# svohr/mixemt

Hardware: AMD Instinct MI355X
Metric: read x hap cells/sec through the EM iteration (EM iters/sec reported beside it as em_iters_per_s), 1000000 reads x 5408 haps in total, whole job (higher is better)
Workload: dtype f64

## Files before the change

### include/mixemt_hip_tuning.h

```cpp
#ifndef MIXEMT_HIP_TUNING_H
#define MIXEMT_HIP_TUNING_H

#include <stddef.h>
#include <stdint.h>

#ifdef __cplusplus
extern "C" {
#endif

struct mxm_em_state;

int mxm_reset_tuning(void);

int mxm_set_timing_events(void *ev_start, void *ev_stop);

int mxm_describe_stream_kernel(int32_t H, int32_t nb, char *buf, size_t len);

int mxm_diag_stream_read(const void *src, size_t bytes, int32_t wg_per_cu, int32_t blocked,
                         void *sink, void *stream);

struct mxm_coded;
int mxm_diag_stream_coded(const struct mxm_coded *c, int32_t H, int32_t wg_per_cu, void *sink, void *stream);

int mxm_diag_stream_quads(const struct mxm_coded *c, int32_t H, int32_t wg_per_cu, void *sink, void *stream);

int mxm_set_progress_callback(void (*fn)(const struct mxm_em_state *state_host, int32_t B, void *user),
                              void *user, int32_t every);

int mxm_set_loop_graph(int32_t mode);

int mxm_set_loop_fused(int32_t mode, int32_t chunk);

int mxm_set_fused_coded_grid(int32_t nwg);

int mxm_set_quad_left_grid(int32_t nwg);

int mxm_set_sparse_long_rows(int32_t on);
int mxm_set_sparse_long_entries(int32_t n);

int mxm_set_quad_encoder(int32_t kind);

int mxm_set_coded_batch_tile(int32_t bt);

int mxm_diag_fused_force_abort(int32_t on);

int mxm_diag_fused_stamps(const void *ws, unsigned long long *out_host);

int mxm_set_batch_tile(int32_t bt);

int mxm_set_compact_restarts(int32_t mode);

#define MXM_SAMPLES_TILE_ROWS 32
int mxm_samples_tile_rows(void);

int mxm_set_min_rows_per_wg(int32_t n);

int mxm_set_sparse_max_distinct(int32_t n);

#ifdef __cplusplus
}
#endif
#endif
```

### mixemt_amd/_lib.py

```python

import ctypes
import os

_PKG = os.path.dirname(os.path.abspath(__file__))
LIB_PATH = os.environ.get("MXM_LIB") or os.path.join(_PKG, "lib", "libmixemt_hip.so")

c_i32, c_i64, c_f64 = ctypes.c_int32, ctypes.c_int64, ctypes.c_double
c_ptr, c_size = ctypes.c_void_p, ctypes.c_size_t


class EmState(ctypes.Structure):
    _fields_ = [("done", c_i32), ("iters", c_i32), ("l1", c_f64), ("ticket", ctypes.c_uint32), ("error", ctypes.c_uint32)]


class Coded(ctypes.Structure):
    _fields_ = [("rec", c_ptr), ("rec_off", c_ptr), ("ndist", c_ptr), ("R", c_i64),
                ("P_rest", c_ptr), ("ldp_rest", c_i64), ("w_rest", c_ptr), ("R_rest", c_i64),
                ("wide_rows", c_ptr), ("n_wide", c_i64),
                ("qrec", c_ptr), ("qoff", c_ptr), ("nquad", c_ptr), ("quad_rows", c_ptr), ("n_quad_rows", c_i64),
                ("byte_rows", c_ptr), ("n_byte_rows", c_i64)]


class SampleTile(ctypes.Structure):
    _fields_ = [("sample", c_i32), ("count", c_i32), ("first", c_i64)]
# ... 80 lines not shown
                                         ctypes.POINTER(EmState)]),
    "mxm_samples_tile_rows": (ctypes.c_int, []),
    "mxm_samples_plan": (c_i64, [c_ptr, c_i32, c_ptr, c_i64, c_ptr]),
    "mxm_samples_workspace_bytes": (c_size, [c_i64, c_i32, c_i32]),
    "mxm_em_iter_samples": (ctypes.c_int, [ctypes.POINTER(Coded), c_ptr, c_i32, c_ptr, c_ptr, c_i32, c_ptr, c_ptr, c_ptr,
                                           c_size, c_ptr]),
    "mxm_em_loop_samples": (ctypes.c_int, [ctypes.POINTER(Coded), c_ptr, c_i32, c_ptr, c_i32, c_ptr, c_ptr, c_ptr, c_ptr,
                                           c_ptr, c_f64, c_i32, c_i32, c_ptr, c_size, c_ptr, ctypes.POINTER(EmState)]),
    "mxm_em_step": (ctypes.c_int, [c_ptr, c_i64, c_ptr, c_ptr, c_i64, c_i32, c_ptr, c_i64, c_i32,
                                   c_ptr, c_ptr, c_size, c_ptr]),
    "mxm_log_normalize": (ctypes.c_int, [c_ptr, c_i32, c_ptr, c_ptr]),
    "mxm_l1_exp_diff": (ctypes.c_int, [c_ptr, c_ptr, c_i32, c_ptr, c_ptr]),
    "mxm_add_scalar": (ctypes.c_int, [c_ptr, c_i64, c_i64, c_i32, c_f64, c_ptr]),
    "mxm_assign_reads": (ctypes.c_int, [c_ptr, c_i64, c_ptr, c_ptr, c_i32, c_i64, c_i32, c_f64, c_ptr, c_ptr]),
    "mxm_diag_stream_read": (ctypes.c_int, [c_ptr, c_size, c_i32, c_i32, c_ptr, c_ptr]),
    "mxm_diag_stream_coded": (ctypes.c_int, [ctypes.POINTER(Coded), c_i32, c_i32, c_ptr, c_ptr]),
    "mxm_diag_stream_quads": (ctypes.c_int, [ctypes.POINTER(Coded), c_i32, c_i32, c_ptr, c_ptr]),
    "mxm_diag_fused_force_abort": (ctypes.c_int, [c_i32]),
    "mxm_set_fused_coded_grid": (ctypes.c_int, [c_i32]),
    "mxm_set_quad_left_grid": (ctypes.c_int, [c_i32]),
    "mxm_set_coded_batch_tile": (ctypes.c_int, [c_i32]),
    "mxm_set_sparse_long_rows": (ctypes.c_int, [c_i32]),
    "mxm_set_quad_encoder": (ctypes.c_int, [c_i32]),
    "mxm_set_sparse_long_entries": (ctypes.c_int, [c_i32]),
    "mxm_diag_fused_stamps": (ctypes.c_int, [c_ptr, ctypes.POINTER(ctypes.c_ulonglong)]),
    "mxm_set_timing_events": (ctypes.c_int, [c_ptr, c_ptr]),
    "mxm_set_batch_tile": (ctypes.c_int, [c_i32]),
    "mxm_encode_signatures": (ctypes.c_int64, [ctypes.c_char_p, c_ptr, c_i64, c_ptr, c_i64, c_ptr, c_ptr, c_ptr,
                                               c_i64]),
    "mxm_aln_encode": (ctypes.c_int, [ctypes.POINTER(AlnColumns), c_ptr, c_i64, c_ptr, c_i32, c_i32, c_i32, c_i32,
                                      ctypes.POINTER(c_ptr)]),
    "mxm_aln_sizes_of": (ctypes.c_int, [c_ptr, ctypes.POINTER(AlnSizes)]),
    "mxm_aln_fetch": (ctypes.c_int, [c_ptr, c_ptr, c_ptr, c_ptr, c_ptr, c_ptr, c_ptr, c_ptr, c_ptr, c_ptr]),
    "mxm_aln_fetch_fragments": (ctypes.c_int, [c_ptr, c_ptr, c_ptr, c_ptr, c_ptr]),
    "mxm_aln_free": (None, [c_ptr]),
    "mxm_bam_read": (ctypes.c_int, [ctypes.c_char_p, c_i32, ctypes.POINTER(c_ptr)]),
    "mxm_bam_sizes_of": (ctypes.c_int, [c_ptr, ctypes.POINTER(BamSizes)]),
    "mxm_bam_columns": (ctypes.c_int, [c_ptr, ctypes.POINTER(AlnColumns)]),
    "mxm_bam_fetch_names": (ctypes.c_int, [c_ptr, c_ptr, c_ptr, c_ptr, c_ptr]),
    "mxm_bam_free": (None, [c_ptr]),
    "mxm_observe_bases": (ctypes.c_int, [ctypes.POINTER(AlnColumns), c_ptr, c_i32, c_i32, c_i64, c_ptr, c_ptr]),
    "mxm_observe_bases_labelled": (ctypes.c_int, [ctypes.POINTER(AlnColumns), c_ptr, c_ptr, c_i32, c_i32, c_i32, c_i64,
                                                  c_ptr, c_ptr]),
    "mxm_consensus": (ctypes.c_int, [c_ptr, c_i32, c_i64, c_i64, c_i64, c_i32, c_ptr, c_ptr, c_ptr, c_ptr]),
    "mxm_new_variants": (ctypes.c_int, [c_ptr, c_i64, c_i32, ctypes.POINTER(c_i32), c_i32, c_i64, c_ptr, c_ptr, c_ptr]),
    "mxm_first_observed": (ctypes.c_int, [ctypes.POINTER(AlnColumns), c_ptr, c_ptr, c_i32, c_i32, c_i32, c_i64, c_ptr,
                                          c_ptr, c_ptr]),
    "mxm_extend_assign": (ctypes.c_int, [ctypes.POINTER(AlnColumns), c_ptr, c_ptr, c_i32, c_i32, ctypes.POINTER(c_i32),
                                         c_i32, c_i32, c_i32, c_i32, c_ptr, c_i64, c_ptr, c_ptr, c_ptr, c_ptr]),
    "mxm_set_compact_restarts": (ctypes.c_int, [c_i32]),
    "mxm_set_loop_graph": (ctypes.c_int, [c_i32]),
    "mxm_set_loop_fused": (ctypes.c_int, [c_i32, c_i32]),
    "mxm_set_progress_callback": (ctypes.c_int, [c_ptr, c_ptr, c_i32]),
    "mxm_set_min_rows_per_wg": (ctypes.c_int, [c_i32]),
    "mxm_reset_tuning": (ctypes.c_int, []),
    "mxm_describe_stream_kernel": (ctypes.c_int, [c_i32, c_i32, ctypes.c_char_p, c_size]),
    "mxm_set_sparse_max_distinct": (ctypes.c_int, [c_i32]),
    "mxm_row_argmax_votes": (ctypes.c_int, [c_ptr, c_i64, c_ptr, c_i64, c_i32, c_ptr, c_ptr,
                                            c_ptr, c_size, c_ptr]),
    "mxm_first_seen": (ctypes.c_int, [c_ptr, c_i64, c_i32, c_ptr, c_ptr]),
    "mxm_gather_columns": (ctypes.c_int, [c_ptr, c_i64, c_i64, c_i32, c_ptr, c_i32, c_ptr, c_i64, c_ptr]),
    "mxm_fold_logaddexp": (ctypes.c_int, [c_ptr, c_i64, ctypes.POINTER(c_ptr), ctypes.POINTER(c_i64), c_i32,
                                          c_i64, c_i32, c_f64, c_ptr]),
}

FINISH_SIGNATURES = {
    "mxm_samples_finish_workspace_bytes": (c_size, [c_i64, c_i32, c_i32]),
    "mxm_votes_samples": (ctypes.c_int, [ctypes.POINTER(Coded), c_ptr, c_i32, c_i32, c_ptr, c_ptr, c_ptr, c_ptr, c_ptr, c_ptr,
                                         c_ptr, c_ptr, c_ptr, c_ptr, c_ptr, c_size, c_ptr]),
    "mxm_gather_columns_samples": (ctypes.c_int, [ctypes.POINTER(Coded), c_ptr, c_i32, c_i32, c_ptr, c_ptr, c_i32, c_ptr,
                                                  c_ptr, c_size, c_ptr]),
    "mxm_em_loop_samples_narrow": (ctypes.c_int, [ctypes.POINTER(Coded), c_ptr, c_i32, c_i32, c_ptr, c_i32, c_ptr, c_ptr,
                                                  c_ptr, c_ptr, c_ptr, c_ptr, c_f64, c_i32, c_i32, c_ptr, c_ptr, c_size,
                                                  c_ptr, ctypes.POINTER(EmState)]),
    "mxm_assign_reads_samples": (ctypes.c_int, [ctypes.POINTER(Coded), c_ptr, c_i32, c_i32, c_ptr, c_i32, c_ptr, c_ptr,
                                                c_ptr, c_ptr, c_ptr, c_ptr, c_f64, c_ptr, c_ptr, c_ptr, c_size, c_ptr]),
}

VARCHECK_SIGNATURES = {
    "mxm_check_variants_samples": (ctypes.c_int, [c_ptr, c_i32, c_i64, c_ptr, c_ptr, c_i32, c_ptr, c_ptr, c_i32, c_i64, c_ptr,
                                                  c_ptr, c_i32, c_f64, c_f64, c_f64, c_i32, c_i32, c_ptr, c_ptr, c_ptr, c_ptr]),
}

ABI_VERSION = 603

PROGRESS_FN = ctypes.CFUNCTYPE(None, ctypes.POINTER(EmState), c_i32, c_ptr)

_lib = None


class MixemtHipError(RuntimeError):
    pass


def load():
    global _lib
    if _lib is not None:
        return _lib
    if not os.path.exists(LIB_PATH):
        raise MixemtHipError(
            "libmixemt_hip.so is not built (%s); run `python -m mixemt_amd.build` -- "
            "there is no CPU fallback for the EM hot path" % LIB_PATH)
    from . import _dev
    lib = ctypes.CDLL(LIB_PATH)
    try:
        lib.mxm_version.restype = ctypes.c_int
        lib.mxm_version.argtypes = []
        have = lib.mxm_version()
    except AttributeError:
        have = None
    if have != ABI_VERSION:
        raise MixemtHipError("%s reports ABI version %s, this binding was written for %d: rebuild with "
                             "`python -m mixemt_amd.build --force`" % (LIB_PATH, have, ABI_VERSION))
    for name, (restype, argtypes) in (list(SIGNATURES.items()) + list(FINISH_SIGNATURES.items())
                                      + list(VARCHECK_SIGNATURES.items())):
        try:
            fn = getattr(lib, name)
        except AttributeError:
            raise MixemtHipError("%s has ABI version %d but lacks %s: rebuild with "
                                 "`python -m mixemt_amd.build --force`" % (LIB_PATH, have, name))
        fn.restype = restype
        fn.argtypes = argtypes
    _lib = lib
    try:
        if _dev.torch is not None and _dev.torch.cuda.is_available():
            lib.mxm_preload()
    except Exception:
        pass
    return lib


def check(rc, what):
    if rc != 0:
        msg = load().mxm_last_error().decode("utf-8", "replace")
        raise ValueError("%s failed (%d): %s" % (what, rc, msg))
```

### mixemt_amd/build.py

```python

import hashlib
import os
import shutil
import subprocess
import sys

_PKG = os.path.dirname(os.path.abspath(__file__))
_ROOT = os.path.dirname(_PKG)
SRC = os.path.join(_PKG, "csrc", "mixemt_hip.hip")
HDRS = [os.path.join(_ROOT, "include", name) for name in ("mixemt_hip.h", "mixemt_hip_tuning.h", "mixemt_hip_samples_finish.h",
                                                           "mixemt_hip_var_check.h")]
LIB_DIR = os.path.join(_PKG, "lib")
LIB = os.path.join(LIB_DIR, "libmixemt_hip.so")
ARCH = "gfx950"


def _hipcc():
    for cand in (os.environ.get("HIPCC"), shutil.which("hipcc"), "/opt/rocm/bin/hipcc"):
        if cand and os.path.exists(cand):
            return cand
    raise RuntimeError("hipcc not found (set HIPCC or add /opt/rocm/bin to PATH)")


def _sources():
    csrc = os.path.dirname(SRC)
    return sorted(os.path.join(csrc, f) for f in os.listdir(csrc) if f.endswith((".hip", ".hpp"))) + HDRS


def _digest(flags):
    h = hashlib.sha256()
    for path in _sources():
        with open(path, "rb") as fin:
            h.update(fin.read())
    h.update(" ".join(flags).encode())
    return h.hexdigest()


def build(force=False, defines=(), verbose=False, out=None):
    global LIB
    if out is not None:
        LIB = os.path.abspath(out)
    flags = ["--offload-arch=%s" % ARCH, "-O3", "-std=c++17", "-shared", "-fPIC", "-Werror=format",
             "-I" + os.path.join(_ROOT, "include"), "-I" + os.path.dirname(SRC)]
    flags += ["-D%s" % d for d in defines]
    stamp = LIB + ".stamp"
    want = _digest(flags)
    if not force and os.path.exists(LIB) and os.path.exists(stamp):
        with open(stamp) as fin:
            if fin.read().strip() == want:
                return LIB
    os.makedirs(os.path.dirname(LIB), exist_ok=True)
    cmd = [_hipcc()] + flags + [SRC, "-o", LIB, "-lz"]
    if verbose:
        sys.stderr.write(" ".join(cmd) + "\n")
    proc = subprocess.run(cmd, stdout=subprocess.PIPE, stderr=subprocess.STDOUT, text=True)
    if proc.returncode != 0:
        raise RuntimeError("hipcc failed:\n" + proc.stdout)
    with open(stamp, "w") as fout:
        fout.write(want + "\n")
    return LIB


if __name__ == "__main__":
    defs = []
    argv = sys.argv[1:]
    i = 0
    while i < len(argv):
        if argv[i] == "-D":
            defs.append(argv[i + 1])
            i += 2
        elif argv[i].startswith("-D"):
            defs.append(argv[i][2:])
            i += 1
        else:
            i += 1
    out_path = argv[argv.index("--out") + 1] if "--out" in argv else None
    print(build(force="--force" in argv, defines=defs, verbose=True, out=out_path))
```

### mixemt_amd/csrc/mixemt_hip.hip

```cpp
#include <hip/hip_runtime.h>
#include <stdint.h>
#include <stdio.h>
#include <stdlib.h>
#include <string.h>
#include <math.h>
#include <algorithm>
#include <atomic>
#include <mutex>
#include <type_traits>
#include <utility>
#include <vector>

#include "mixemt_hip.h"
#include "mixemt_hip_tuning.h"

#include "common.hpp"
#include "aln_encode.hpp"
#include "bam_reader.hpp"
#include "coded_kernels.hpp"
#include "quad_kernels.hpp"
#include "quad_batched_kernels.hpp"
#include "build_kernels.hpp"
#include "build_lut_kernels.hpp"
#include "build_sparse_kernels.hpp"
#include "em_kernels.hpp"
#include "estep_kernels.hpp"
#include "aux_kernels.hpp"
#include "records_kernels.hpp"
#include "fused_kernels.hpp"
#include "fused_cols_kernels.hpp"
#include "fused_coded_kernels.hpp"
#include "fused_narrow_kernels.hpp"
#include "samples_kernels.hpp"
#include "samples_finish_kernels.hpp"
#include "exchange.hpp"
#include "aln_walk.hpp"
#include "observe_kernels.hpp"
#include "var_check_kernels.hpp"
#include "assemble_kernels.hpp"


struct mxm_em_state;
typedef void (*mxm_progress_fn)(const mxm_em_state *state_host, int32_t B, void *user);
struct mxm_tuning {
    int sparse_maxd = -1;
    int min_rows_per_wg = 8;
    int compact_restarts = 2;
    int max_bt = 4;
    int loop_graph = -1;
    int loop_fused = -1;
    int fused_chunk = 0;
    int fused_cols = 1;
    int fused_coded_wg = 0;
    int quad_left_wg = 0;
    int sparse_long_entries = 5120;
    int quad_encoder = 1;
    int sparse_long = 1;
    int coded_bt = 3;
    int fused_force_abort = 0;
    double fused_cells = 1.0e8;
    hipEvent_t ev_start = nullptr, ev_stop = nullptr;
    mxm_progress_fn progress = nullptr;
    void *progress_user = nullptr;
    int progress_every = 10;
};
static std::mutex g_tune_mu;
static mxm_tuning g_tune;
static thread_local mxm_tuning T;
#define MXM_ENTER() do { std::lock_guard<std::mutex> lk_(g_tune_mu); T = g_tune; } while (0)
template <typename F>
static int tune_set(F f) {
    std::lock_guard<std::mutex> lk(g_tune_mu);
    f(g_tune);
    return 0;
}
extern "C" int mxm_reset_tuning(void) {
    return tune_set([](mxm_tuning &t) { t = mxm_tuning(); });
}

static inline int clamp_grid(int64_t want, int cap) {
    if (want < 1) want = 1;
    return (int)(want < cap ? want : cap);
}

static inline int64_t part_ld(int H) { return ((int64_t)H + 1) & ~(int64_t)1; }

static hipError_t raise_dynamic_lds(const void *kernel, size_t bytes, const char *name) {
    const hipError_t e = hipFuncSetAttribute(kernel, hipFuncAttributeMaxDynamicSharedMemorySize, (int)bytes);
    if (e != hipSuccess)
        snprintf(g_err, sizeof(g_err), "%s: cannot opt into %zu bytes of dynamic LDS: %s", name, bytes,
                 hipGetErrorString(e));
    return e;
}
static int dynamic_lds_ok(const void *kernel, size_t bytes, const char *name, const char *who = nullptr, int H = 0,
                          const char *too_wide = nullptr) {
    if (too_wide != nullptr && bytes > 150 * 1024) return fail(-1, "%s: H=%d %s", who, H, too_wide);
    if (bytes > 60 * 1024 && raise_dynamic_lds(kernel, bytes, name) != hipSuccess) return -2;
    return 0;
}

#define RC_TRY(expr)                                                                         \
    do {                                                                                     \
        const int rc_ = (expr);                                                              \
        if (rc_ != 0) return rc_;                                                            \
    } while (0)

template <int MAX, typename F>
static bool dispatch_width(int n, F &&f) {
    if constexpr (MAX < 1) {
        return false;
    } else {
        if (n != MAX) return dispatch_width<MAX - 1>(n, f);
        f(std::integral_constant<int, MAX>{});
        return true;
    }
}

extern "C" int mxm_version(void) { return MXM_VERSION; }
extern "C" const char *mxm_last_error(void) { return g_err; }

extern "C" int mxm_linear_supported(int32_t H) {
    return (H >= MXM_LINEAR_MIN_H && H <= 8192) ? 1 : 0;
}

static size_t fused_sync_bytes() { return (sizeof(fused_sync) + 255) & ~(size_t)255; }
static size_t fused_snapshot_bytes(int H, int B) {
    return ((size_t)3 * B * H * sizeof(double) + (size_t)B * sizeof(mxm_em_state) + 255) & ~(size_t)255;
}
static size_t fused_rows_bytes(int H, int nwg) { return (size_t)(nwg + 2) * part_ld(H) * sizeof(double); }
static size_t fused_cols_bytes(int64_t R, int nwg) {
    const size_t ldz = (size_t)((R + 1) & ~(int64_t)1);
    return ((size_t)(nwg + 1) * ldz + 2 * (size_t)nwg) * sizeof(double);
}

extern "C" size_t mxm_workspace_bytes(int64_t R, int32_t H, int32_t B) {
    const size_t tiles = (size_t)MXM_MAX_WG * MXM_MAX_BT * (size_t)part_ld(H) * sizeof(double);
    size_t fused = fused_rows_bytes(H, MXM_MAX_WG);
    if (R > 0 && R <= (int64_t)FCOLS_MAX_RPT * FCOLS_THREADS) fused = std::max(fused, fused_cols_bytes(R, MXM_MAX_WG));
    fused += fused_sync_bytes() + fused_snapshot_bytes(H, B > 0 ? B : 1) + 512;
// ... 226 lines not shown
        rec_off == nullptr || ndist == nullptr || rowmax == nullptr || stats == nullptr)
        return fail(-1, "mxm_build_em_records: record buffer (16-byte aligned, >= one record) and output arrays required");
    spb_records out;
    out.rec = rec;
    out.rec_cap = (long long)rec_bytes;
    out.rec_off = rec_off;
    out.ndist = ndist;
    out.rowmax = rowmax;
    out.stats = reinterpret_cast<unsigned long long *>(stats);
    out.ldc = coded_ld(H);
    return build_sparse_impl("mxm_build_em_records", maj, lhit, lmiss, mk_ptr, mk_hap, mk_base, row_ptr, site, obs, order,
                             R, H, S, M, ldm, &out, fallback, n_fallback, (hipStream_t)stream);
}

template <typename ST>
static int linearize_wide(const double *M, int64_t ldm, int64_t R, int H, ST *P, int64_t ldp, double *rowmax,
                          hipStream_t s) {
    const int nch = (H / 2 + 255) / 256;
    int cap = num_cu() * 2 < MXM_MAX_WG ? num_cu() * 2 : MXM_MAX_WG;
    const int nwg = clamp_grid((R + 1) / 2, cap);
    const bool ok = dispatch_width<16>(nch, [&](auto n) {
        hipLaunchKernelGGL((linearize_wide_kernel<decltype(n)::value, ST>), dim3(nwg), dim3(256), 0, s, M, ldm, R, H, P, ldp, rowmax);
    });
    return ok ? 0 : 1;
}

static inline bool wide_rows_ok(const void *M, int64_t ldm, int H) {
    return ((H & 1) == 0) && ((ldm & 1) == 0) && ((reinterpret_cast<uintptr_t>(M) & 15) == 0) && H >= 64 && H <= 8192;
}

extern "C" int mxm_linearize(const double *M, int64_t ldm, int64_t R, int32_t H, double *P, int64_t ldp,
                             double *rowmax, void *stream) {
    if (R < 0 || H <= 0) return fail(-1, "mxm_linearize: bad shape");
    if (ldm < H || ldp < H || (ldp & 1)) return fail(-1, "mxm_linearize: ldp must be even and >= H (ldp=%lld)", (long long)ldp);
    if (R == 0) return 0;
    if (wide_rows_ok(M, ldm, H) && (reinterpret_cast<uintptr_t>(P) & 15) == 0 &&
        linearize_wide<double>(M, ldm, R, (int)H, P, ldp, rowmax, (hipStream_t)stream) == 0) {
        HIP_TRY(hipGetLastError());
        return 0;
    }
    const int grid = clamp_grid(R, num_cu() * 8);
    hipLaunchKernelGGL(linearize_kernel, dim3(grid), dim3(ROW_THREADS), 0, (hipStream_t)stream, M, ldm, R,
                       (int)H, P, ldp, rowmax);
    HIP_TRY(hipGetLastError());
    return 0;
}

extern "C" int mxm_set_timing_events(void *ev_start, void *ev_stop) {
    return tune_set([=](mxm_tuning &t) { t.ev_start = (hipEvent_t)ev_start; t.ev_stop = (hipEvent_t)ev_stop; });
}

extern "C" int mxm_set_min_rows_per_wg(int32_t n) {
    if (n < 1) return fail(-1, "mxm_set_min_rows_per_wg: n < 1");
    return tune_set([n](mxm_tuning &t) { t.min_rows_per_wg = n; });
}

extern "C" int mxm_set_compact_restarts(int32_t mode) {
    return tune_set([mode](mxm_tuning &t) { t.compact_restarts = mode < 0 ? 0 : (mode > 2 ? 2 : mode); });
}

extern "C" int mxm_set_batch_tile(int32_t bt) {
    if (bt < 1 || bt > 4) return fail(-1, "mxm_set_batch_tile: tile must be 1..4");
    return tune_set([bt](mxm_tuning &t) { t.max_bt = bt; });
}

extern "C" int mxm_set_fused_coded_grid(int32_t nwg) {
    return tune_set([nwg](mxm_tuning &t) { t.fused_coded_wg = nwg > 0 ? nwg : 0; });
}

extern "C" int mxm_set_sparse_long_rows(int32_t on) {
    return tune_set([on](mxm_tuning &t) { t.sparse_long = on ? 1 : 0; });
}
extern "C" int mxm_set_sparse_long_entries(int32_t n) {
    return tune_set([n](mxm_tuning &t) { t.sparse_long_entries = n > 0 ? n : 0; });
}
extern "C" int mxm_set_coded_batch_tile(int32_t bt) {
    if (bt != 1 && bt != 3) return fail(-1, "mxm_set_coded_batch_tile: 1 or 3, got %d", bt);
    return tune_set([bt](mxm_tuning &t) { t.coded_bt = bt; });
}
extern "C" int mxm_set_quad_encoder(int32_t kind) {
    if (kind != 0 && kind != 1) return fail(-1, "mxm_set_quad_encoder: 0 or 1, got %d", kind);
    return tune_set([kind](mxm_tuning &t) { t.quad_encoder = kind; });
}
extern "C" int mxm_set_quad_left_grid(int32_t nwg) {
    return tune_set([nwg](mxm_tuning &t) { t.quad_left_wg = nwg > 0 ? nwg : 0; });
}

extern "C" int mxm_diag_fused_force_abort(int32_t on) {
    return tune_set([on](mxm_tuning &t) { t.fused_force_abort = on ? 1 : 0; });
}

#ifndef MXM_V1_THREADS
#define MXM_V1_THREADS 256
#endif
#ifndef MXM_V1_NBUF
#define MXM_V1_NBUF 2
#endif
#ifndef MXM_V1_WG_PER_CU
#define MXM_V1_WG_PER_CU 2
#endif
#ifndef MXM_V2_THREADS
#define MXM_V2_THREADS 512
#endif
#ifndef MXM_V2_NBUF
#define MXM_V2_NBUF 2
#endif
#ifndef MXM_V3_THREADS
#define MXM_V3_THREADS 512
#endif
#ifndef MXM_V3_NBUF
#define MXM_V3_NBUF 2
#endif
#ifndef MXM_V4_THREADS
#define MXM_V4_THREADS 512
#endif
#ifndef MXM_V4_NBUF
#define MXM_V4_NBUF 2
#endif
#ifndef MXM_V2_PREG
#define MXM_V2_PREG 1
#endif
#ifndef MXM_V3_PREG
#define MXM_V3_PREG 2
#endif
#ifndef MXM_V4_PREG
#define MXM_V4_PREG 2
#endif
#ifndef MXM_V1B_THREADS
#define MXM_V1B_THREADS 512
#endif
#ifndef MXM_V1B_NBUF
#define MXM_V1B_NBUF 3
#endif
#define MXM_MAX_COL2 4096
#define MXM_LDS_BUDGET (156 * 1024)

static inline int variant_threads(int nb) {
    return nb == 1 ? MXM_V1_THREADS : (nb == 2 ? MXM_V2_THREADS : (nb == 3 ? MXM_V3_THREADS : MXM_V4_THREADS));
}
static inline int variant_preg(int nb) {
    return nb == 1 ? 1 : (nb == 2 ? MXM_V2_PREG : (nb == 3 ? MXM_V3_PREG : MXM_V4_PREG));
}

static size_t batch_lds_bytes(int H, int nb) {
    const int threads = variant_threads(nb);
    const int nch = ((H + 1) / 2 + threads - 1) / threads;
    return (size_t)(nb - variant_preg(nb)) * nch * threads * 16;
}

static bool batch_fits(int H, int nb) {
    if (nb <= 1) return true;
    static const int max_nch[MXM_MAX_BT + 1] = {0, 16, 8, 7, 6};
    const int threads = variant_threads(nb);
    const int nch = ((H + 1) / 2 + threads - 1) / threads;
    return nch <= max_nch[nb] && batch_lds_bytes(H, nb) <= MXM_LDS_BUDGET;
}

template <int THREADS, int NCH, int BT, int NBUF, int PREG>
static int launch_wide(const double *P, int64_t ldp, const double *w, const double *props, int64_t R,
                       int H, int grid, double *partial, int64_t ldpart,
                       const mxm_em_state *state, mxm_slots slots, hipStream_t stream) {
    if constexpr (NCH * THREADS > MXM_MAX_COL2) {
        return fail(-1, "mxm_em_iter: H=%d outside the linear kernel's range", H);
    } else {
        const size_t lds = (size_t)(BT - PREG) * NCH * THREADS * sizeof(d2);
        RC_TRY(dynamic_lds_ok(reinterpret_cast<const void *>(&em_iter_wide_kernel<THREADS, NCH, BT, NBUF, PREG>), lds, "em_iter_wide_kernel"));
// ... 180 lines not shown
        hipLaunchKernelGGL((estep_global_kernel<true>), dim3(nwg), dim3(ROW_THREADS), 0, stream, M, ldm, w, ln_props, R, H,
                           (double *)nullptr, (int64_t)0, 0, partial, ldpart, state, (const int64_t *)nullptr);
        HIP_TRY(hipGetLastError());
    } else if (H <= MXM_NARROW_MAX_H) {
        const int rc = launch_narrow<true>(M, ldm, w, ln_props, R, H, (double *)nullptr, (int64_t)0, 0, partial, ldpart,
                                           state, stream, &nwg);
        if (rc != 0) return rc;
    } else {
        nwg = clamp_grid(R, num_cu() * 2 < MXM_MAX_WG ? num_cu() * 2 : MXM_MAX_WG);
        RC_TRY(dynamic_lds_ok(reinterpret_cast<const void *>(&estep_log_kernel<true>), lds, "estep_log_kernel"));
        hipLaunchKernelGGL((estep_log_kernel<true>), dim3(nwg), dim3(ROW_THREADS), lds, stream, M, ldm, w, ln_props,
                           R, H, (double *)nullptr, (int64_t)0, 0, partial, ldpart, state);
        HIP_TRY(hipGetLastError());
    }
    return reduce_one(partial, nwg, H, colsum, state, stream);
}

extern "C" int mxm_em_iter(const double *M, int64_t ldm, const double *P, int64_t ldp, const double *w,
                           const double *props, const double *ln_props, int64_t R, int32_t H, int32_t B,
                           const mxm_em_state *state, double *colsum, void *ws, size_t ws_bytes, void *stream) {
    MXM_ENTER();
    if (R <= 0 || H <= 0 || B <= 0) return fail(-1, "mxm_em_iter: bad shape R=%lld H=%d", (long long)R, H);
    if (ws == nullptr || ws_bytes < mxm_workspace_bytes(R, H, B)) return fail(-1, "mxm_em_iter: workspace too small");
    if (P != nullptr && ((ldp & 1) || ldp < H)) return fail(-1, "mxm_em_iter: ldp must be even and >= H");
    if (M != nullptr && ldm < H) return fail(-1, "mxm_em_iter: ldm < H");
    const bool linear = (P != nullptr) && mxm_linear_supported(H);
    int max_bt = linear ? T.max_bt : 1;
    while (max_bt > 1 && !batch_fits((int)H, max_bt)) --max_bt;
    for (int b = 0; b < B;) {
        const int left = B - b;
        const int passes = (left + max_bt - 1) / max_bt;
        const int nb = (left + passes - 1) / passes;
        const mxm_em_state *st = state ? state + b : nullptr;
        int rc;
        if (linear)
            rc = em_iter_linear_tile(P, ldp, w, props, R, (int)H, nb, slots_from(b), state, colsum, (double *)ws,
                                     (hipStream_t)stream, b == 0);
        else
            rc = em_iter_log_one(M, ldm, w, ln_props ? ln_props + (int64_t)b * H : nullptr, R, (int)H, st,
                                 colsum + (int64_t)b * H, (double *)ws, (hipStream_t)stream);
        if (rc != 0) return rc;
        b += nb;
    }
    return 0;
}

extern "C" int mxm_linearize_f32(const double *M, int64_t ldm, int64_t R, int32_t H, float *P, int64_t ldp,
                                 double *rowmax, void *stream) {
    if (R < 0 || H <= 0) return fail(-1, "mxm_linearize_f32: bad shape");
    if (ldm < H || ldp < H || (ldp & 3)) return fail(-1, "mxm_linearize_f32: ldp must be a multiple of 4 and >= H (ldp=%lld)", (long long)ldp);
    if (R == 0) return 0;
    if (wide_rows_ok(M, ldm, H) && (reinterpret_cast<uintptr_t>(P) & 7) == 0 && (ldp & 1) == 0 &&
        linearize_wide<float>(M, ldm, R, (int)H, P, ldp, rowmax, (hipStream_t)stream) == 0) {
        HIP_TRY(hipGetLastError());
        return 0;
    }
    const int grid = clamp_grid(R, num_cu() * 8);
    hipLaunchKernelGGL(linearize_f32_kernel, dim3(grid), dim3(ROW_THREADS), 0, (hipStream_t)stream, M, ldm, R, (int)H,
                       P, ldp, rowmax);
    HIP_TRY(hipGetLastError());
    return 0;
}

extern "C" int mxm_em_iter_f32(const float *P, int64_t ldp, const double *w, const double *props, int64_t R,
                               int32_t H, int32_t B, const mxm_em_state *state, double *colsum, void *ws,
                               size_t ws_bytes, void *stream) {
    MXM_ENTER();
    if (R <= 0 || H <= 0 || B <= 0) return fail(-1, "mxm_em_iter_f32: bad shape R=%lld H=%d", (long long)R, H);
    if (!mxm_linear_supported(H)) return fail(-1, "mxm_em_iter_f32: H=%d outside the linear kernel's range", H);
    if (P == nullptr || (ldp & 3) || ldp < H) return fail(-1, "mxm_em_iter_f32: ldp must be a multiple of 4 and >= H");
    if (ws == nullptr || ws_bytes < mxm_workspace_bytes(R, H, B)) return fail(-1, "mxm_em_iter_f32: workspace too small");
    for (int b = 0; b < B; ++b) {
        const int rc = em_iter_f32_one(P, ldp, w, props + (int64_t)b * H, R, (int)H, state ? state + b : nullptr,
                                       colsum + (int64_t)b * H, (double *)ws, (hipStream_t)stream, b == 0);
        if (rc != 0) return rc;
    }
    return 0;
}

extern "C" size_t mxm_coded_bytes(int64_t R, int32_t H) { return mxm_record_bytes(R, H); }

extern "C" int mxm_encode_rows(const double *M, int64_t ldm, int64_t R, int32_t H, uint8_t *rec, size_t rec_bytes,
                               int64_t *rec_off, int32_t *ndist, double *rowmax, int64_t *stats, void *stream) {
    if (R <= 0 || H <= 0 || ldm < H) return fail(-1, "mxm_encode_rows: bad shape R=%lld H=%d", (long long)R, H);
    if (!mxm_linear_supported(H) || (reinterpret_cast<uintptr_t>(M) & 7) != 0)
        return fail(-1, "mxm_encode_rows: needs H in [65, 8192] (H=%d ldm=%lld)", H, (long long)ldm);
    if (rec == nullptr || (reinterpret_cast<uintptr_t>(rec) & 15) || rec_bytes < (size_t)coded_ld(H) + 16 * ENC_MAX_CODES)
        return fail(-1, "mxm_encode_rows: record buffer missing, unaligned or smaller than one record");
    if (rec_off == nullptr || ndist == nullptr || rowmax == nullptr || stats == nullptr)
        return fail(-1, "mxm_encode_rows: output arrays required");
    hipStream_t s = (hipStream_t)stream;
    HIP_TRY(hipMemsetAsync(stats, 0, 2 * sizeof(int64_t), s));
    const int ldc = coded_ld(H);
    const int nch = (ldc / 4 + ENC_THREADS - 1) / ENC_THREADS;
    const int grid = clamp_grid(R, num_cu() * 4);
    const int grid_w = clamp_grid((R + 31) / 32, num_cu() * 3);
    const bool ok = dispatch_width<8>(nch, [&](auto n) {
        constexpr int NCH = decltype(n)::value;
        unsigned long long *st = reinterpret_cast<unsigned long long *>(stats);
        hipLaunchKernelGGL((encode_rows_kernel<NCH>), dim3(grid), dim3(ENC_THREADS), 0, s, M, ldm, R, (int)H, ldc, rec,
                           (int64_t)rec_bytes, rec_off, ndist, rowmax, st);
        hipLaunchKernelGGL((encode_wide_rows_kernel<NCH>), dim3(grid_w), dim3(ENC_THREADS), 0, s, M, ldm, R, (int)H, ldc, rec,
                           (int64_t)rec_bytes, rec_off, ndist, rowmax, st);
    });
    if (!ok) return fail(-1, "mxm_encode_rows: H=%d outside the kernel's range", H);
    HIP_TRY(hipGetLastError());
    return 0;
}

static int coded_check(const mxm_coded *c, int32_t H, const char *who) {
    if (c == nullptr || c->R <= 0 || H <= 0 || !mxm_linear_supported(H))
        return fail(-1, "%s: bad coded matrix (rows %lld, H %d)", who, (long long)(c ? c->R : 0), H);
    if (c->rec == nullptr || c->rec_off == nullptr || c->ndist == nullptr) return fail(-1, "%s: coded matrix arrays missing", who);
    if (c->R_rest < 0 || (c->R_rest > 0 && (c->P_rest == nullptr || c->ldp_rest < H || (c->ldp_rest & 1) ||
                                            (reinterpret_cast<uintptr_t>(c->P_rest) & 15))))
        return fail(-1, "%s: the dense rest needs 16-byte aligned rows with an even ld >= H", who);
    if (c->n_wide < 0 || (c->n_wide > 0 && c->wide_rows == nullptr)) return fail(-1, "%s: n_wide > 0 needs wide_rows", who);
    if (c->qrec != nullptr) {
        if (c->qoff == nullptr || c->nquad == nullptr || c->n_quad_rows < 0 || c->n_byte_rows < 0 ||
            (c->n_quad_rows > 0 && c->quad_rows == nullptr) || (c->n_byte_rows > 0 && c->byte_rows == nullptr) ||
            (reinterpret_cast<uintptr_t>(c->qrec) & 31))
            return fail(-1, "%s: quad dictionary arrays missing (or qrec not 32-byte aligned)", who);
        if (c->n_quad_rows + c->n_byte_rows + c->n_wide + c->R_rest != c->R)
            return fail(-1, "%s: quad_rows + byte_rows + wide_rows + the dense rest must be all %lld rows", who, (long long)c->R);
    }
    return 0;
}

static int rest_check(const char *who, int32_t H, const double *M_rest, int64_t ldm_rest, const int64_t *rest_rows, int64_t n_rest) {
    if (n_rest < 0 || (n_rest > 0 && (M_rest == nullptr || rest_rows == nullptr || ldm_rest < H)))
        return fail(-1, "%s: the rows without a record need M_rest, rest_rows and ldm_rest >= H", who);
    return 0;
}

extern "C" size_t mxm_quad_bytes(int64_t R, int32_t H) {
    (void)H;
    constexpr size_t largest = QUAD_CODE_BYTES + QUAD_MAX * 32, per_piece = (size_t)QUAD_CHUNK / largest;
    return R > 0 ? (((size_t)R + per_piece - 1) / per_piece + 5120) * (size_t)QUAD_CHUNK : 0;
}

extern "C" int mxm_expand_tables(const uint8_t *maj, const int32_t *mk_ptr, const uint16_t *mk_hap, const uint8_t *mk_base,
                                 const uint8_t *map256, int32_t S, int32_t H, int64_t lde, uint8_t *out, void *stream) {
    if (maj == nullptr || mk_ptr == nullptr || mk_hap == nullptr || mk_base == nullptr || out == nullptr || S <= 0 || H <= 0 || lde < H)
        return fail(-1, "mxm_expand_tables: bad arguments");
    hipLaunchKernelGGL(expand_tables_kernel, dim3(clamp_grid(S, num_cu() * 8)), dim3(256), 0, (hipStream_t)stream, maj, mk_ptr, mk_hap,
                       mk_base, map256, (int)S, (int)H, lde, out);
    HIP_TRY(hipGetLastError());
    return 0;
}

extern "C" size_t mxm_quad_lists_scratch_bytes(int64_t R) {
    return R > 0 ? (size_t)((R + QLIST_CHUNK - 1) / QLIST_CHUNK) * 2 * sizeof(long long) : 0;
}

extern "C" int mxm_quad_lists(const int32_t *ndist, const int32_t *nquad, int64_t R, int64_t *quad_rows, int64_t *byte_rows,
                              int64_t *counts, void *scratch, size_t scratch_bytes, void *stream) {
    MXM_ENTER();
    if (ndist == nullptr || nquad == nullptr || R <= 0 || quad_rows == nullptr || byte_rows == nullptr || counts == nullptr)
        return fail(-1, "mxm_quad_lists: bad arguments");
    if (scratch == nullptr || scratch_bytes < mxm_quad_lists_scratch_bytes(R)) return fail(-1, "mxm_quad_lists: scratch too small");
    const int64_t nchunk = (R + QLIST_CHUNK - 1) / QLIST_CHUNK;
    if (nchunk > 0x7fffffff) return fail(-1, "mxm_quad_lists: too many rows");
    hipStream_t s = (hipStream_t)stream;
    long long *cc = static_cast<long long *>(scratch);
    hipLaunchKernelGGL(quad_list_count_kernel, dim3((unsigned)nchunk), dim3(QLIST_THREADS), 0, s, ndist, nquad, R, cc);
    hipLaunchKernelGGL(quad_list_scan_kernel, dim3(1), dim3(QLIST_THREADS), 0, s, cc, nchunk, reinterpret_cast<long long *>(counts));
    hipLaunchKernelGGL(quad_list_fill_kernel, dim3((unsigned)nchunk), dim3(QLIST_THREADS), 0, s, ndist, nquad, R, cc, quad_rows, byte_rows);
    HIP_TRY(hipGetLastError());
    return 0;
}

extern "C" int mxm_build_quads(const mxm_coded *c, int32_t H, uint8_t *qrec, size_t qrec_bytes, int64_t *qoff, int32_t *nquad,
                               uint64_t *stats, void *stream) {
    MXM_ENTER();
    if (c == nullptr || c->R <= 0 || c->rec == nullptr || c->rec_off == nullptr || c->ndist == nullptr || !mxm_linear_supported(H))
        return fail(-1, "mxm_build_quads: bad coded matrix (rows %lld, H %d)", (long long)(c ? c->R : 0), H);
    if (qoff == nullptr || nquad == nullptr || stats == nullptr || (qrec == nullptr && qrec_bytes > 0) ||
        (reinterpret_cast<uintptr_t>(qrec) & 31))
        return fail(-1, "mxm_build_quads: qoff, nquad, stats and a 32-byte aligned qrec required");
    const int ldc = coded_ld(H);
    if (ldc / 4 > 8 * QUAD_THREADS) return fail(-1, "mxm_build_quads: H=%d beyond eight quads per thread", H);
    HIP_TRY(hipMemsetAsync(stats, 0, 2 * sizeof(uint64_t), (hipStream_t)stream));
    if (T.quad_encoder == 1 && ldc / 4 <= 64 * QW_K)
        hipLaunchKernelGGL(quad_encode_wave_kernel, dim3(clamp_grid((c->R + QW_WAVES - 1) / QW_WAVES, std::min(num_cu() * QW_MIN_WAVES, 5120 / QW_WAVES))), dim3(QUAD_THREADS),
                           0, (hipStream_t)stream, c->rec, c->rec_off, c->ndist, ldc, (int)H, c->R, qrec,
                           (unsigned long long)qrec_bytes, qoff, nquad, reinterpret_cast<unsigned long long *>(stats));
    else
        hipLaunchKernelGGL(quad_encode_kernel, dim3(clamp_grid(c->R, num_cu() * 8)), dim3(QUAD_THREADS), 0, (hipStream_t)stream,
// ... 1669 lines not shown
```

Baseline: 871.8 billion.

## Add list-based row encoder that dedups adjacent values before hash probing

Adds a new row-encoding kernel, enabled by default. Each wave first compacts runs of equal adjacent values into a per-wave LDS list using DPP, ballot and mbcnt, then inserts only those distinct keys into the shared hash table. It falls back to per-strip processing when the list overflows. The grid is sized from occupancy queries, and the next row is prefetched while the current one is encoded. The goal is fewer atomic CAS hash probes during encoding, at the cost of more LDS, extra code complexity and added register pressure.

After: 871.8 billion (median of 2 runs). No clear change (-0.0%).

```diff
diff --git a/include/mixemt_hip_row_encoder.h b/include/mixemt_hip_row_encoder.h
--- /dev/null
+++ b/include/mixemt_hip_row_encoder.h
@@ -0,0 +1,15 @@
+#ifndef MIXEMT_HIP_ROW_ENCODER_H
+#define MIXEMT_HIP_ROW_ENCODER_H
+
+#include <stdint.h>
+
+#ifdef __cplusplus
+extern "C" {
+#endif
+
+int mxm_set_row_encoder(int32_t kind);
+
+#ifdef __cplusplus
+}
+#endif
+#endif
diff --git a/include/mixemt_hip_tuning.h b/include/mixemt_hip_tuning.h
--- a/include/mixemt_hip_tuning.h
+++ b/include/mixemt_hip_tuning.h
@@ -60,4 +60,7 @@
 #ifdef __cplusplus
 }
 #endif
+
+#include "mixemt_hip_row_encoder.h"
+
 #endif
diff --git a/mixemt_amd/_lib.py b/mixemt_amd/_lib.py
--- a/mixemt_amd/_lib.py
+++ b/mixemt_amd/_lib.py
@@ -186,6 +186,10 @@
                                                   c_ptr, c_i32, c_f64, c_f64, c_f64, c_i32, c_i32, c_ptr, c_ptr, c_ptr, c_ptr]),
 }
 
+ROW_ENCODER_SIGNATURES = {
+    "mxm_set_row_encoder": (ctypes.c_int, [c_i32]),
+}
+
 ABI_VERSION = 603
 
 PROGRESS_FN = ctypes.CFUNCTYPE(None, ctypes.POINTER(EmState), c_i32, c_ptr)
@@ -217,7 +221,7 @@
         raise MixemtHipError("%s reports ABI version %s, this binding was written for %d: rebuild with "
                              "`python -m mixemt_amd.build --force`" % (LIB_PATH, have, ABI_VERSION))
     for name, (restype, argtypes) in (list(SIGNATURES.items()) + list(FINISH_SIGNATURES.items())
-                                      + list(VARCHECK_SIGNATURES.items())):
+                                      + list(VARCHECK_SIGNATURES.items()) + list(ROW_ENCODER_SIGNATURES.items())):
         try:
             fn = getattr(lib, name)
         except AttributeError:
diff --git a/mixemt_amd/build.py b/mixemt_amd/build.py
--- a/mixemt_amd/build.py
+++ b/mixemt_amd/build.py
@@ -9,7 +9,7 @@
 _ROOT = os.path.dirname(_PKG)
 SRC = os.path.join(_PKG, "csrc", "mixemt_hip.hip")
 HDRS = [os.path.join(_ROOT, "include", name) for name in ("mixemt_hip.h", "mixemt_hip_tuning.h", "mixemt_hip_samples_finish.h",
-                                                           "mixemt_hip_var_check.h")]
+                                                           "mixemt_hip_var_check.h", "mixemt_hip_row_encoder.h")]
 LIB_DIR = os.path.join(_PKG, "lib")
 LIB = os.path.join(LIB_DIR, "libmixemt_hip.so")
 ARCH = "gfx950"
diff --git a/mixemt_amd/csrc/mixemt_hip.hip b/mixemt_amd/csrc/mixemt_hip.hip
--- a/mixemt_amd/csrc/mixemt_hip.hip
+++ b/mixemt_amd/csrc/mixemt_hip.hip
@@ -20,6 +20,7 @@
 #include "coded_kernels.hpp"
 #include "quad_kernels.hpp"
 #include "quad_batched_kernels.hpp"
+#include "row_encoder_kernels.hpp"
 #include "build_kernels.hpp"
 #include "build_lut_kernels.hpp"
 #include "build_sparse_kernels.hpp"
@@ -55,6 +56,7 @@
     int quad_left_wg = 0;
     int sparse_long_entries = 5120;
     int quad_encoder = 1;
+    int row_encoder = 1;
     int sparse_long = 1;
     int coded_bt = 3;
     int fused_force_abort = 0;
@@ -447,6 +449,10 @@
     if (kind != 0 && kind != 1) return fail(-1, "mxm_set_quad_encoder: 0 or 1, got %d", kind);
     return tune_set([kind](mxm_tuning &t) { t.quad_encoder = kind; });
 }
+extern "C" int mxm_set_row_encoder(int32_t kind) {
+    if (kind != 0 && kind != 1) return fail(-1, "mxm_set_row_encoder: 0 or 1, got %d", kind);
+    return tune_set([kind](mxm_tuning &t) { t.row_encoder = kind; });
+}
 extern "C" int mxm_set_quad_left_grid(int32_t nwg) {
     return tune_set([nwg](mxm_tuning &t) { t.quad_left_wg = nwg > 0 ? nwg : 0; });
 }
@@ -793,6 +799,7 @@
 
 extern "C" int mxm_encode_rows(const double *M, int64_t ldm, int64_t R, int32_t H, uint8_t *rec, size_t rec_bytes,
                                int64_t *rec_off, int32_t *ndist, double *rowmax, int64_t *stats, void *stream) {
+    MXM_ENTER();
     if (R <= 0 || H <= 0 || ldm < H) return fail(-1, "mxm_encode_rows: bad shape R=%lld H=%d", (long long)R, H);
     if (!mxm_linear_supported(H) || (reinterpret_cast<uintptr_t>(M) & 7) != 0)
         return fail(-1, "mxm_encode_rows: needs H in [65, 8192] (H=%d ldm=%lld)", H, (long long)ldm);
@@ -806,15 +813,25 @@
     const int nch = (ldc / 4 + ENC_THREADS - 1) / ENC_THREADS;
     const int grid = clamp_grid(R, num_cu() * 4);
     const int grid_w = clamp_grid((R + 31) / 32, num_cu() * 3);
+    hipError_t occ_err = hipSuccess;
     const bool ok = dispatch_width<8>(nch, [&](auto n) {
         constexpr int NCH = decltype(n)::value;
         unsigned long long *st = reinterpret_cast<unsigned long long *>(stats);
-        hipLaunchKernelGGL((encode_rows_kernel<NCH>), dim3(grid), dim3(ENC_THREADS), 0, s, M, ldm, R, (int)H, ldc, rec,
-                           (int64_t)rec_bytes, rec_off, ndist, rowmax, st);
+        if (T.row_encoder == 1) {
+            int per_cu = 0;
+            occ_err = hipOccupancyMaxActiveBlocksPerMultiprocessor(&per_cu, encode_rows_list_kernel<NCH>, ENC_THREADS, 0);
+            if (occ_err != hipSuccess) return;
+            const int grid_l = clamp_grid(R, num_cu() * (per_cu > 0 ? per_cu : 1));
+            hipLaunchKernelGGL((encode_rows_list_kernel<NCH>), dim3(grid_l), dim3(ENC_THREADS), 0, s, M, ldm, R, (int)H, ldc, rec,
+                               (int64_t)rec_bytes, rec_off, ndist, rowmax, st);
+        } else
+            hipLaunchKernelGGL((encode_rows_kernel<NCH>), dim3(grid), dim3(ENC_THREADS), 0, s, M, ldm, R, (int)H, ldc, rec,
+                               (int64_t)rec_bytes, rec_off, ndist, rowmax, st);
         hipLaunchKernelGGL((encode_wide_rows_kernel<NCH>), dim3(grid_w), dim3(ENC_THREADS), 0, s, M, ldm, R, (int)H, ldc, rec,
                            (int64_t)rec_bytes, rec_off, ndist, rowmax, st);
     });
     if (!ok) return fail(-1, "mxm_encode_rows: H=%d outside the kernel's range", H);
+    HIP_TRY(occ_err);
     HIP_TRY(hipGetLastError());
     return 0;
 }
diff --git a/mixemt_amd/csrc/row_encoder_kernels.hpp b/mixemt_amd/csrc/row_encoder_kernels.hpp
--- /dev/null
+++ b/mixemt_amd/csrc/row_encoder_kernels.hpp
@@ -0,0 +1,250 @@
+#ifndef MIXEMT_ROW_ENCODER_KERNELS_HPP
+#define MIXEMT_ROW_ENCODER_KERNELS_HPP
+
+#define ENC_LIST 256
+#ifndef ENC_LIST_WAVES
+#define ENC_LIST_WAVES(NCH) ((NCH) <= 6 ? 3 : 2)
+#endif
+
+template <int NCH>
+__global__ __launch_bounds__(ENC_THREADS, ENC_LIST_WAVES(NCH)) void encode_rows_list_kernel(
+    const double *__restrict__ M, int64_t ldm, int64_t R, int H, int ldc, uint8_t *__restrict__ rec, int64_t rec_cap,
+    int64_t *__restrict__ rec_off, int32_t *__restrict__ ndist, double *__restrict__ rowmax,
+    unsigned long long *__restrict__ stats) {
+    constexpr int NW = ENC_THREADS / 64;
+    constexpr int SLOTS = ENC_SLOTS;
+    constexpr int MAXC = ENC_MAX_CODES;
+    constexpr int SPT = SLOTS / ENC_THREADS;
+    static_assert(ENC_LIST >= 256, "a strip's 256 cells must fit a wave's list");
+    __shared__ unsigned long long s_key[SLOTS];
+    __shared__ unsigned long long s_list[NW * (ENC_LIST + 64)];
+    __shared__ unsigned short s_code[SLOTS + NW * ENC_LIST];
+    __shared__ unsigned long long s_val[MAXC];
+    __shared__ double s_red[NW];
+    __shared__ int s_wcnt[NW];
+    __shared__ int s_flag, s_n;
+    __shared__ long long s_off;
+    const int t = threadIdx.x, lane = t & 63, wv = t >> 6;
+    typedef unsigned int u4 __attribute__((ext_vector_type(4)));
+    unsigned long long *const my_list = s_list + wv * (ENC_LIST + 64);
+    unsigned short *const my_ref = s_code + SLOTS + wv * ENC_LIST;
+    int tr = t;
+
+    double x[NCH][4];
+    auto load_row = [&](int64_t rr, bool live) {
+        const auto rsrc = __builtin_amdgcn_make_buffer_rsrc(const_cast<double *>(M + rr * ldm), 0, live ? H * 8 : 0, 0x00020000);
+        quad_static_for<NCH>([&](auto K) {
+            constexpr int k = decltype(K)::value;
+            const int off = (t + k * ENC_THREADS) * 32;
+            const d2 a = __builtin_bit_cast(d2, (u4)__builtin_amdgcn_raw_buffer_load_b128(rsrc, off, 0, 2));
+            const d2 b = __builtin_bit_cast(d2, (u4)__builtin_amdgcn_raw_buffer_load_b128(rsrc, off, 16, 2));
+            x[k][0] = a.x;
+            x[k][1] = a.y;
+            x[k][2] = b.x;
+            x[k][3] = b.y;
+        });
+    };
+
+    unsigned int pk[NCH][2];
+    auto list_strip = [&](auto K, int base) -> int {
+        constexpr int k = decltype(K)::value;
+        constexpr bool inside = k < NCH - 1;
+        const int c0 = 4 * (tr + k * ENC_THREADS);
+        const int ln = tr & 63;
+        unsigned long long key[4];
+        bool valid[4], head[4];
+#pragma unroll
+        for (int e = 0; e < 4; ++e) {
+            key[e] = (unsigned long long)__double_as_longlong(x[k][e]);
+            valid[e] = inside || c0 + e < H;
+        }
+        const unsigned int left_lo = (unsigned int)__builtin_amdgcn_update_dpp(0, (int)(unsigned int)key[3], 0x138, 0xf, 0xf, false);
+        const unsigned int left_hi = (unsigned int)__builtin_amdgcn_update_dpp(0, (int)(unsigned int)(key[3] >> 32), 0x138, 0xf, 0xf, false);
+        const unsigned long long left = ((unsigned long long)left_hi << 32) | left_lo;
+        head[0] = valid[0] && (ln == 0 || key[0] != left);
+#pragma unroll
+        for (int e = 1; e < 4; ++e) head[e] = valid[e] && key[e] != key[e - 1];
+        int at = base, total = 0;
+#pragma unroll
+        for (int e = 0; e < 4; ++e) {
+            const unsigned long long votes = __builtin_amdgcn_ballot_w64(head[e]);
+            at = (int)__builtin_amdgcn_mbcnt_hi((unsigned int)(votes >> 32), __builtin_amdgcn_mbcnt_lo((unsigned int)votes, (unsigned int)at));
+            total += __builtin_popcountll(votes);
+        }
+        unsigned int ref[4];
+#pragma unroll
+        for (int e = 0; e < 4; ++e) {
+            at += head[e] ? 1 : 0;
+            const bool put = head[e] && at <= ENC_LIST;
+            my_list[put ? at - 1 : ENC_LIST + ln] = key[e];
+            ref[e] = (valid[e] && at <= ENC_LIST) ? (unsigned int)(at - 1) : 0u;
+        }
+        pk[k][0] = ref[0] | (ref[1] << 16);
+        pk[k][1] = ref[2] | (ref[3] << 16);
+        return total;
+    };
+    auto probe_list = [&](int n) {
+        for (int i0 = 0; i0 < n; i0 += 64) {
+            if (__builtin_amdgcn_readfirstlane(__hip_atomic_load(&s_flag, __ATOMIC_RELAXED, __HIP_MEMORY_SCOPE_WORKGROUP)) != 0) break;
+            const int i = i0 + (tr & 63);
+            if (i < n) {
+                const unsigned long long key = my_list[i];
+                if (key == ENC_EMPTY) s_flag = 1;
+                unsigned int h = (unsigned int)((key ^ (key >> 29)) * 0x9E3779B97F4A7C15ull >> 40) & (SLOTS - 1);
+                for (int probes = 0;; ++probes) {
+                    const unsigned long long old = atomicCAS(&s_key[h], ENC_EMPTY, key);
+                    if (old == ENC_EMPTY) {
+                        if (atomicAdd(&s_n, 1) >= MAXC) s_flag = 1;
+                        break;
+                    }
+                    if (old == key) break;
+                    h = (h + 1) & (SLOTS - 1);
+                    if (probes >= SLOTS) {
+                        s_flag = 1;
+                        break;
+                    }
+                }
+                my_ref[i] = (unsigned short)h;
+            }
+        }
+    };
+
+#pragma unroll
+    for (int q = 0; q < SPT; ++q) s_key[t + q * ENC_THREADS] = ENC_EMPTY;
+    if (t == 0) {
+        s_flag = 0;
+        s_n = 0;
+    }
+    int64_t r = blockIdx.x;
+    load_row(r, r < R);
+    __syncthreads();
+    const int cbytes = ldc;
+    for (; r < R; r += gridDim.x) {
+        asm volatile("" : "+v"(tr));
+        if (H & 1) {
+            const double tail = M[r * ldm + (H - 1)];
+            quad_static_for<NCH>([&](auto K) {
+                constexpr int k = decltype(K)::value;
+                if (4 * (tr + k * ENC_THREADS) == H - 1) x[k][0] = tail;
+                if (4 * (tr + k * ENC_THREADS) + 2 == H - 1) x[k][2] = tail;
+            });
+        }
+        double m = -INFINITY;
+        quad_static_for<NCH>([&](auto K) {
+            constexpr int k = decltype(K)::value;
+#pragma unroll
+            for (int e = 0; e < 4; ++e)
+                if (k < NCH - 1 || 4 * (tr + k * ENC_THREADS) + e < H) m = fmax(m, x[k][e]);
+        });
+        m = wave_max(m);
+        if (lane == 0) s_red[wv] = m;
+
+        int n_list = 0;
+        quad_static_for<NCH>([&](auto K) { n_list += list_strip(K, n_list); });
+        const bool by_strip = n_list > ENC_LIST;
+        if (!by_strip) {
+            wave_lds_fence();
+            probe_list(n_list);
+        } else {
+            asm volatile("" : "+v"(tr));
+            quad_static_for<NCH>([&](auto K) {
+                constexpr int k = decltype(K)::value;
+                wave_lds_fence();
+                const int n = list_strip(K, 0);
+                wave_lds_fence();
+                probe_list(n);
+                wave_lds_fence();
+                const unsigned int a = my_ref[pk[k][0] & 0xffffu], b = my_ref[pk[k][0] >> 16];
+                const unsigned int c = my_ref[pk[k][1] & 0xffffu], d = my_ref[pk[k][1] >> 16];
+                pk[k][0] = a | (b << 16);
+                pk[k][1] = c | (d << 16);
+            });
+        }
+        __syncthreads();
+        asm volatile("" : "+v"(tr));
+        const bool dense = __hip_atomic_load(&s_flag, __ATOMIC_RELAXED, __HIP_MEMORY_SCOPE_WORKGROUP) != 0;
+        const int D = s_n;
+        const int64_t bytes = (int64_t)cbytes + 16 * (int64_t)D;
+        const bool coded = !dense && D <= MAXC;
+        long long got = -1;
+        unsigned int zero = 0;
+        asm volatile("" : "+v"(zero));
+#ifdef ENC_LIST_FIXED_SLOTS
+        if (t == 0 && coded) got = (long long)(r + zero) * (cbytes + 16 * MAXC);
+#else
+        if (t == 0 && coded) got = (long long)atomicAdd(stats + zero, (unsigned long long)bytes);
+#endif
+        const int64_t rn = r + gridDim.x;
+        load_row(rn < R ? rn : r, rn < R);
+        const double shift_m = fmax(fmax(s_red[0], s_red[1]), fmax(s_red[2], s_red[3]));
+        const double shift = isfinite(shift_m) ? shift_m : 0.0;
+        unsigned long long kk[SPT];
+        int cnt = 0;
+#pragma unroll
+        for (int j = 0; j < SPT; ++j) {
+            kk[j] = s_key[SPT * tr + j];
+            cnt += (kk[j] != ENC_EMPTY) ? 1 : 0;
+        }
+        const int incl = wave_inclusive_scan_i32(cnt);
+        if (lane == 63) s_wcnt[wv] = incl;
+        __syncthreads();
+        int code = incl - cnt;
+#pragma unroll
+        for (int q = 0; q < NW; ++q)
+            if (q < wv) code += s_wcnt[q];
+#pragma unroll
+        for (int j = 0; j < SPT; ++j) {
+            if (kk[j] != ENC_EMPTY) {
+                if (code < MAXC) {
+                    s_code[SPT * tr + j] = (unsigned short)code;
+                    s_val[code] = kk[j];
+                }
+                ++code;
+                s_key[SPT * tr + j] = ENC_EMPTY;
+            }
+        }
+        if (t == 0) {
+            if (got >= 0 && got + bytes > rec_cap) got = -1;
+            s_off = got;
+        }
+        __syncthreads();
+        const long long off = s_off;
+        if (off >= 0) {
+            if (!by_strip) {
+                for (int i = tr & 63; i < n_list; i += 64) my_ref[i] = s_code[my_ref[i]];
+                wave_lds_fence();
+            }
+            const unsigned short *codes_of = by_strip ? s_code : my_ref;
+            quad_static_for<NCH>([&](auto K) {
+                constexpr int k = decltype(K)::value;
+                const int c0 = 4 * (tr + k * ENC_THREADS);
+                constexpr bool inside = k < NCH - 1;
+                if (inside || c0 < ldc) {
+                    unsigned int cd[4];
+                    cd[0] = (inside || c0 + 0 < H) ? (unsigned int)codes_of[pk[k][0] & 0xffffu] : 0u;
+                    cd[1] = (inside || c0 + 1 < H) ? (unsigned int)codes_of[pk[k][0] >> 16] : 0u;
+                    cd[2] = (inside || c0 + 2 < H) ? (unsigned int)codes_of[pk[k][1] & 0xffffu] : 0u;
+                    cd[3] = (inside || c0 + 3 < H) ? (unsigned int)codes_of[pk[k][1] >> 16] : 0u;
+                    reinterpret_cast<unsigned int *>(rec + off)[tr + k * ENC_THREADS] = cd[0] | (cd[1] << 8) | (cd[2] << 16) | (cd[3] << 24);
+                }
+            });
+            if (tr < D) {
+                double *tbl = reinterpret_cast<double *>(rec + off + cbytes);
+                const double mval = __longlong_as_double((long long)s_val[tr]);
+                tbl[tr] = exp(mval - shift);
+                tbl[D + tr] = mval;
+            }
+        }
+        if (t == 0) {
+            rowmax[r] = shift;
+            ndist[r] = (off >= 0) ? D : 0;
+            rec_off[r] = (off >= 0) ? off : 0;
+            if (off < 0) atomicAdd(&stats[1], 1ull);
+            s_flag = 0;
+            s_n = 0;
+        }
+        __syncthreads();
+    }
+}
+
+#endif
diff --git a/profiles/encoder/compare.py b/profiles/encoder/compare.py
--- /dev/null
+++ b/profiles/encoder/compare.py
@@ -0,0 +1,55 @@
+import glob
+import json
+import os
+import statistics
+
+HERE = os.path.dirname(os.path.abspath(__file__))
+FIELDS = (("coded_storage.encode_ms", "ms", "lower"), ("value", "cells/s", "control"), ("coded_storage.kernel_ms", "ms", "control"),
+          ("coded_storage.quads.kernel_ms", "ms", "control"), ("coded_storage.max_rel_dcolsum", "", "same"),
+          ("coded_storage.quads.max_rel_dcolsum", "", "same"), ("sanity_ok", "", "same"))
+
+
+def field(rec, dotted):
+    for scope in (rec, rec.get("extra", {})):
+        cur = scope
+        try:
+            for key in dotted.split("."):
+                cur = cur[key]
+            return cur
+        except (KeyError, TypeError):
+            continue
+    return None
+
+
+def runs(tag):
+    out = []
+    for path in sorted(glob.glob(os.path.join(HERE, "bench_%s_*.json" % tag))):
+        lines = [ln for ln in open(path) if ln.lstrip().startswith("{")]
+        out.append(json.loads(lines[-1]))
+    return out
+
+
+def main():
+    parent, branch = runs("parent"), runs("branch")
+    print("| field | parent (3 runs) | branch (3 runs) | verdict |")
+    print("|---|---|---|---|")
+    for dotted, unit, kind in FIELDS:
+        a, b = [field(r, dotted) for r in parent], [field(r, dotted) for r in branch]
+        if kind == "same":
+            verdict = "the same" if all(v == a[0] for v in a + b) else "DIFFERENT"
+            show = lambda vals: ", ".join(repr(v) for v in vals)
+        else:
+            show = lambda vals: ", ".join("%.4g" % v for v in vals) + " " + unit
+            if kind == "lower":
+                verdict = ("branch max %.4g < parent min %.4g: %.1f %% less (medians)"
+                           % (max(b), min(a), 100.0 * (1.0 - statistics.median(b) / statistics.median(a)))
+                           if max(b) < min(a) else "NOT separated")
+            else:
+                med = statistics.median(a)
+                lo, hi = min(a) - 0.02 * med, max(a) + 0.02 * med
+                verdict = "inside the parent's spread" if lo <= statistics.median(b) <= hi else "OUTSIDE the parent's spread"
+        print("| `%s` | %s | %s | %s |" % (dotted, show(a), show(b), verdict))
+
+
+if __name__ == "__main__":
+    main()
```
